# alipay/MMLRec-A-Unified-Multi-Task-and-Multi-Scenario-Learning-Benchmark-for-Recommendation

Measured on AMD Instinct MI355X. Metric: train-step samples/sec, MMoE AliExpress-shape batch, higher is better.
Workload: dtype f32 (GEMMs: fp32-equivalent emulation on the 16-bit MFMA pipe with f32 accumulate -- two scaled fp16 planes per operand where the operand magnitudes travel with the tensors (batches >= 32 768), else three bf16 planes; max-norm error vs float64 3.3e-7 / 4.7e-7, fp32 MFMA 4.3e-7); 1 GPU; mmoe_ae30: 30 sparse fields, 12.49M rows (1e+07-row top table), E=8, mmoe 4 experts, experts [256, 128], gates [64], towers [64], adam lr 0.005; batch_per_gpu=65536, global_batch=65536, index_dist=zipf, table_update=dense_exact, dense_update_schedule=one launch after the scatter, gradients read for marked rows only, hip_graph=True, scatter_mode=deterministic, streams=1, early_fork=0, tables=single GPU

## Files before the change

mmlrec-a-unified-multi-task-and-multi-scenario-learning-benchmark-for-recommendation_amd/csrc/gemm.hip:

```cpp
#include "common.hpp"
#include "gemm_route.hpp"
#include "lds_async.hpp"
#include "reduce.hpp"

#include <stdlib.h>

#include <type_traits>

namespace mml {

using f32x16 = __attribute__((ext_vector_type(16))) float;

constexpr int PITCH_RC = BK + 4;
constexpr int PITCH_NRC = 128 + 4;

struct Source {
  const float* A;
  const float* B;
  int64_t lda, ldb;
  int32_t Kred;
  int32_t vecA, vecB;
  const uint32_t* amaxA;
  const uint32_t* amaxB;
};
// ... 1446 lines not shown
      if (amo) {
        const uint32_t a = lds0 + (uint32_t)(PSTAGES * STG + 256 + tid) * 4u;
        uint32_t v;
        asm volatile("ds_read_b32 %0, %1\n\ts_waitcnt lgkmcnt(0)" : "=v"(v) : "v"(a) : "memory");
        if (v) atomicMax(amo + (blockIdx.x & (MML_AMAX_WORDS - 1)), v);
      }
      uint32_t* const amo2 = K7 ? L.p[tid].amax_out2 : nullptr;
      if (amo2) {
        const uint32_t a = lds0 + (uint32_t)(PSTAGES * STG + 256 + MML_MAX_GROUP + tid) * 4u;
        uint32_t v;
        asm volatile("ds_read_b32 %0, %1\n\ts_waitcnt lgkmcnt(0)" : "=v"(v) : "v"(a) : "memory");
        if (v) atomicMax(amo2 + (blockIdx.x & (MML_AMAX_WORDS - 1)), v);
      }
    }
  }
}

static GemmEnv& gemm_env() {
  static GemmEnv env = [] {
    auto num = [](const char* name, int dflt) {
      const char* e = getenv(name);
      return e ? atoi(e) : dflt;
    };
    auto off = [](const char* name) {
      const char* e = getenv(name);
      return (e && e[0] == '0') ? 0 : 1;
    };
    GemmEnv v = GEMM_ENV_DEFAULT;
    const char* m = getenv("MMLREC_GEMM_MODE");
    v.mode = (m && m[0] >= '0' && m[0] <= '3') ? m[0] - '0' : 4;
    v.panel_on = off("MMLREC_GEMM_PANEL");
    v.ws_on = off("MMLREC_GEMM_WS");
    v.nt_mode = num("MMLREC_GEMM_NT", 1);
    if (v.nt_mode < 0 || v.nt_mode > 3) v.nt_mode = 1;
    v.nt_per_cu = num("MMLREC_NT_PER_CU", 2) == 1 ? 1 : 2;
    v.glds_on = off("MMLREC_GEMM_GLDS");
    v.planes_on = num("MMLREC_GEMM_PLANES", 1);
    v.force_bn = num("MMLREC_GEMM_BN", 0);
    v.wgrad_pad = num("MMLREC_WGRAD_LDS_PAD", 0);
    return v;
  }();
  const char* e = getenv("MMLREC_GEMM_OS");
  env.os_on = (e && e[0] == '0') ? 0 : 1;
  return env;
}

static thread_local char g_last_kernel[96] = "";
static int noted(int rc, const GemmLaunch& g, bool report) {
  if (rc == MML_OK && report) memcpy(g_last_kernel, g.symbol, sizeof(g_last_kernel));
  return rc;
}
static_assert(sizeof(g_last_kernel) == sizeof(GemmLaunch::symbol), "symbol buffers");

template <int EPI, bool A_, bool B_, int N_, bool C_>
static void launch_pipe(const GemmLaunch& G, const Launch& L, hipStream_t st) {
  const dim3 g(G.grid), b(256);
  const size_t dyn = (size_t)G.dyn_lds;
#ifdef MML_LAB
  if (G.bpl) MML_LAUNCH((gemm_pipe_kernel<A_, B_, N_, EPI, MML_LAB_EMU, false, (EPI != EPI_SLAB && MML_LAB_EMU == 2)>), g, b, dyn, st, L);
  else MML_LAUNCH((gemm_pipe_kernel<A_, B_, N_, EPI, MML_LAB_EMU, false>), g, b, dyn, st, L);
#else
  if constexpr (EPI != EPI_SLAB && ((EPI == EPI_FWD) == (B_)) && (EPI == EPI_FWD || N_ == 64)) {
    if (G.k7) {
      if (G.emu == 2 && G.bpl) MML_LAUNCH((gemm_pipe_kernel<A_, B_, N_, EPI, 2, false, true, true>), g, b, dyn, st, L);
      else if (G.emu == 2) MML_LAUNCH((gemm_pipe_kernel<A_, B_, N_, EPI, 2, false, false, true>), g, b, dyn, st, L);
      else MML_LAUNCH((gemm_pipe_kernel<A_, B_, N_, EPI, 3, false, false, true>), g, b, dyn, st, L);
      return;
// ... 45 lines not shown
}

static void put_shape(Problem& P, const TileProb& t) {
  P.M = t.M; P.N = t.N; P.src0 = t.src0; P.nsrc = t.nsrc; P.tiles_n = t.tiles_n; P.tile0 = t.tile0; P.vec_out = t.vec_out;
}
static void put_shape(Source& S, const TileSrc& t) { S.Kred = t.Kred; S.vecA = t.vecA; S.vecB = t.vecB; }

}

using namespace mml;

extern "C" int mml_gemm_set_mode(int32_t mode) {
  MML_REQUIRE(mode == 0 || mode == 1 || mode == 2 || mode == 3 || mode == 4,
              "mml_gemm_set_mode: mode must be 0 (fp32 MFMA), 1 (bf16 operands, reduced precision), 2 / 4 (auto: fp32 "
              "emulated from two scaled fp16 planes where the operand magnitudes are given, else from three bf16 "
              "planes) or 3 (three bf16 planes on every LDS-DMA launch)");
  gemm_env().mode = mode;
  return MML_OK;
}

extern "C" int mml_gemm_get_mode(void) { return gemm_env().mode; }

extern "C" int mml_gemm_set_panel(int32_t on) {
  gemm_env().panel_on = on ? 1 : 0;
  return MML_OK;
}

extern "C" int mml_gemm_set_ws(int32_t on) {
  gemm_env().ws_on = on ? 1 : 0;
  return MML_OK;
}

extern "C" int mml_gemm_set_nt(int32_t on) {
  MML_REQUIRE(on >= 0 && on <= 3, "mml_gemm_set_nt: 0 (off), 1 (every qualifying launch: default), 2 (launches of >= 16 tiles) "
              "or 3 (lab: every qualifying launch on gemm_ntd_kernel)");
  gemm_env().nt_mode = on;
  return MML_OK;
}

extern "C" int mml_gemm_set_wgrad_lds_pad(int32_t bytes) {
  MML_REQUIRE(bytes >= 0 && bytes <= 64 * 1024, "mml_gemm_set_wgrad_lds_pad: bytes outside [0, 65536]");
  gemm_env().wgrad_pad = bytes;
  return MML_OK;
}

extern "C" const char* mml_gemm_last_kernel(void) { return g_last_kernel; }

extern "C" int mml_gemm_nt_serves(const mml_gemm_wgrad_desc* desc) { return (desc && nt_problem_ok(*desc)) ? 1 : 0; }

extern "C" int mml_gemm_os_serves(const mml_gemm_dgrad_desc* d, int32_t n) {
  return (n > 0 && planes_kernels_on(gemm_env()) && os_serves(d, n, gemm_env())) ? 1 : 0;
}

extern "C" int mml_gemm_planes_cut(const mml_planes_desc* d, int32_t n, mml_stream_t stream) {
  MML_REQUIRE(n >= 0 && (n == 0 || d), "mml_gemm_planes_cut: bad descriptor array");
  int i = 0;
  while (i < n) {
    PlanesLaunch L{};
    int64_t items = 0;
    while (i < n && L.n < PLANES_PER_LAUNCH) {
      const mml_planes_desc& q = d[i];
      MML_REQUIRE(q.W && q.planes && q.kexp && q.rows >= 0 && q.cols >= 0 && q.ld >= q.cols,
                  "mml_gemm_planes_cut: matrix %d malformed", i);
      MML_REQUIRE(q.layout == MML_PLANES_ROWS || q.layout == MML_PLANES_COLS, "mml_gemm_planes_cut: layout of matrix %d", i);
      const int64_t ldp = q.ldp ? q.ldp : q.ld;
      MML_REQUIRE(q.layout == MML_PLANES_ROWS ? ldp >= (q.cols + 15) / 16 * 16 : (q.rows % 16 == 0 && ldp >= q.cols),
                  "mml_gemm_planes_cut: matrix %d: the planes pitch cannot hold the reduction extent rounded up to 16 "
                  "(ROWS), or the row count is not a multiple of 16 (COLS)", i);
// ... 227 lines not shown
```

mmlrec-a-unified-multi-task-and-multi-scenario-learning-benchmark-for-recommendation_amd/csrc/gemm_nt.hip:

```cpp
#include "common.hpp"
#include "gemm_route.hpp"
#include "lds_async.hpp"

namespace mml {

typedef float f32x16 __attribute__((ext_vector_type(16)));
typedef short s16x4 __attribute__((ext_vector_type(4)));
typedef short s16x8 __attribute__((ext_vector_type(8)));
typedef __attribute__((address_space(3))) s16x4 lds_s16x4_t;

constexpr int NT_PLANE = NT_STEP * 128;
constexpr int NT_STAGE = 4 * NT_PLANE;

struct NtProblem {
  const float* dC;
  const float* A;
  float* ws;
  float* ws_bias;
  const uint32_t* amax_dc;
  const uint32_t* amax_a;
  int64_t lddc, lda;
  int32_t N, K, ntiles, ktiles;
};
struct NtLaunch {
  NtProblem p[NT_MAX_GROUP];
  int32_t n_prob, steps, slabs, tiles;
};

__device__ __forceinline__ uint32_t nt_amax_load(const uint32_t* p) {
  uint32_t m = 0;
#pragma unroll
  for (int i = 0; i < MML_AMAX_WORDS; ++i) m = p[i] > m ? p[i] : m;
  return m;
}
__device__ __forceinline__ int nt_scale_exp(uint32_t bits) {
  const int e = (int)((bits >> 23) & 0xffu);
  if (e == 255) return 0;
  const int k = 141 - e;
  return k > 110 ? 110 : (k < -110 ? -110 : k);
}
__device__ __forceinline__ float nt_pow2(int k) { return __uint_as_float((uint32_t)(127 + k) << 23); }

__device__ __forceinline__ int nt_swz32(int row) { return ((row & 3) << 2) | ((row >> 2) & 3); }

__device__ __forceinline__ f16x8 nt_frag32(const uint16_t* img, int lo_off, int hi_off) {
  const s16x4 lo = __builtin_amdgcn_ds_read_tr16_b64_v4i16((lds_s16x4_t*)(img + lo_off));
  const s16x4 hi = __builtin_amdgcn_ds_read_tr16_b64_v4i16((lds_s16x4_t*)(img + hi_off));
  const s16x8 v = {lo.x, lo.y, lo.z, lo.w, hi.x, hi.y, hi.z, hi.w};
  return __builtin_bit_cast(f16x8, v);
}
__device__ __forceinline__ int nt_frag_off(int chunk0, int lane, int t) {
  const int g = lane >> 4, hh = g >> 1, q = (lane & 15) >> 2, p = lane & 3;
  const int ch = chunk0 + 2 * (g & 1) + (p >> 1);
  const int row = 8 * hh + 4 * t + q;
  return row * 128 + ((ch ^ nt_swz32(row)) << 3) + 4 * (p & 1);
}

__device__ __forceinline__ void nt_cut4(const float4& x, const float s, uint2& h, uint2& l) {
  typedef float f32x2 __attribute__((ext_vector_type(2)));
  float r0, r1, r2, r3;
  uint32_t h0, h1, l0, l1;
  const f32x2 x01 = {x.x, x.y}, x23 = {x.z, x.w}, ss = {s, s};
  f32x2 y01, y23;
  asm("v_pk_mul_f32 %0, %1, %2" : "=v"(y01) : "v"(x01), "s"(ss));
  asm("v_pk_mul_f32 %0, %1, %2" : "=v"(y23) : "v"(x23), "s"(ss));
  asm("v_cvt_pk_f16_f32 %0, %1, %2" : "=v"(h0) : "v"(y01.x), "v"(y01.y));
  asm("v_cvt_pk_f16_f32 %0, %1, %2" : "=v"(h1) : "v"(y23.x), "v"(y23.y));
  asm("v_fma_mix_f32 %0, %1, %2, -%3 op_sel:[0,0,0] op_sel_hi:[0,0,1]" : "=v"(r0) : "v"(x.x), "s"(s), "v"(h0));
  asm("v_fma_mix_f32 %0, %1, %2, -%3 op_sel:[0,0,1] op_sel_hi:[0,0,1]" : "=v"(r1) : "v"(x.y), "s"(s), "v"(h0));
  asm("v_fma_mix_f32 %0, %1, %2, -%3 op_sel:[0,0,0] op_sel_hi:[0,0,1]" : "=v"(r2) : "v"(x.z), "s"(s), "v"(h1));
  asm("v_fma_mix_f32 %0, %1, %2, -%3 op_sel:[0,0,1] op_sel_hi:[0,0,1]" : "=v"(r3) : "v"(x.w), "s"(s), "v"(h1));
  asm("v_cvt_pk_f16_f32 %0, %1, %2" : "=v"(l0) : "v"(r0), "v"(r1));
  asm("v_cvt_pk_f16_f32 %0, %1, %2" : "=v"(l1) : "v"(r2), "v"(r3));
  h = make_uint2(h0, h1);
  l = make_uint2(l0, l1);
}

__global__ __launch_bounds__(256, 2) void gemm_nt_kernel(const NtLaunch L) {
  __shared__ __attribute__((aligned(16))) uint16_t lds[2 * NT_STAGE];
  const int tid = threadIdx.x, lane = tid & 63, w = __builtin_amdgcn_readfirstlane(tid >> 6);
  const int wn = w >> 1, wk = w & 1;
  const int id = xcd_remap(blockIdx.x, gridDim.x);
  const int slab = id / L.tiles;
  int t = id - slab * L.tiles;
  int pi = 0;
  while (t >= L.p[pi].ntiles * L.p[pi].ktiles) t -= L.p[pi].ntiles * L.p[pi].ktiles, ++pi;
  const NtProblem& P = L.p[pi];
  const int nt = t / P.ktiles, kt = t - nt * P.ktiles;
  const int n0 = nt * 128, k0 = kt * 128;
  const int per = (L.steps + L.slabs - 1) / L.slabs;
  const int s_begin = slab * per, s_end = min(L.steps, s_begin + per);
  const bool want_bias = P.ws_bias != nullptr && kt == 0;

  int kC = nt_scale_exp(nt_amax_load(P.amax_dc)), kA = nt_scale_exp(nt_amax_load(P.amax_a));
  {
    const int over = kC + kA - 126, under = -126 - (kC + kA);
    if (over > 0) { kC -= (over + 1) >> 1; kA -= over >> 1; }
    if (under > 0) { kC += (under + 1) >> 1; kA += under >> 1; }
  }
  kC = __builtin_amdgcn_readfirstlane(kC);
  kA = __builtin_amdgcn_readfirstlane(kA);
  const float sC = nt_pow2(kC), sA = nt_pow2(kA), inv = nt_pow2(-(kC + kA));

  f32x16 acc[2][2];
#pragma unroll
  for (int i = 0; i < 2; ++i)
#pragma unroll
    for (int j = 0; j < 2; ++j)
#pragma unroll
      for (int r = 0; r < 16; ++r) acc[i][j][r] = 0.f;
  float4 bsum = make_float4(0.f, 0.f, 0.f, 0.f);

  const int c4 = tid & 31, r8 = tid >> 5;
  const bool colC = n0 + 4 * c4 < P.N, colA = k0 + 4 * c4 < P.K;
  const uint32_t tC = (uint32_t)(((int64_t)r8 * P.lddc + (colC ? n0 + 4 * c4 : 0)) * 4);
  const uint32_t tA = (uint32_t)(((int64_t)r8 * P.lda + (colA ? k0 + 4 * c4 : 0)) * 4);
  float4 rc0[4], ra0[4], rc1[4], ra1[4];
  const int last = s_end - 1;
  auto load_step = [&](int st, float4 (&rc)[4], float4 (&ra)[4]) __attribute__((always_inline)) {
    st = st > last ? last : st;
    const char* const bC = reinterpret_cast<const char*>(P.dC + (int64_t)st * NT_STEP * P.lddc);
    const char* const bA = reinterpret_cast<const char*>(P.A + (int64_t)st * NT_STEP * P.lda);
#pragma unroll
    for (int p = 0; p < 4; ++p) {
      rc[p] = *reinterpret_cast<const float4*>(bC + (int64_t)(8 * p) * P.lddc * 4 + tC);
      ra[p] = *reinterpret_cast<const float4*>(bA + (int64_t)(8 * p) * P.lda * 4 + tA);
    }
  };
  auto store_step = [&](uint16_t* stage, const float4 (&rc)[4], const float4 (&ra)[4], const float count) __attribute__((always_inline)) {
#pragma unroll
    for (int p = 0; p < 4; ++p) {
      const int row = r8 + 8 * p;
      const int off = row * 128 + (((c4 >> 1) ^ nt_swz32(row)) << 3) + 4 * (c4 & 1);
      uint2 h, l;
      nt_cut4(rc[p], sC, h, l);
      *reinterpret_cast<uint2*>(stage + off) = h;
      *reinterpret_cast<uint2*>(stage + NT_PLANE + off) = l;
      nt_cut4(ra[p], sA, h, l);
      *reinterpret_cast<uint2*>(stage + 2 * NT_PLANE + off) = h;
      *reinterpret_cast<uint2*>(stage + 3 * NT_PLANE + off) = l;
      bsum.x = fmaf(rc[p].x, count, bsum.x); bsum.y = fmaf(rc[p].y, count, bsum.y);
      bsum.z = fmaf(rc[p].z, count, bsum.z); bsum.w = fmaf(rc[p].w, count, bsum.w);
    }
  };
  int offC[2][2], offA[2][2];
#pragma unroll
  for (int i = 0; i < 2; ++i)
#pragma unroll
    for (int t2 = 0; t2 < 2; ++t2) {
      offC[i][t2] = nt_frag_off(wn * 8 + i * 4, lane, t2);
      offA[i][t2] = nt_frag_off(wk * 8 + i * 4, lane, t2);
    }
  auto compute = [&](const uint16_t* cur) __attribute__((always_inline)) {
#pragma unroll
    for (int sub = 0; sub < 2; ++sub) {
      const uint16_t* const b0 = cur + sub * 16 * 128;
      f16x8 ah[2], al[2], bh[2], bl[2];
#pragma unroll
      for (int i = 0; i < 2; ++i) {
        ah[i] = nt_frag32(b0, offC[i][0], offC[i][1]);
        al[i] = nt_frag32(b0 + NT_PLANE, offC[i][0], offC[i][1]);
        bh[i] = nt_frag32(b0 + 2 * NT_PLANE, offA[i][0], offA[i][1]);
        bl[i] = nt_frag32(b0 + 3 * NT_PLANE, offA[i][0], offA[i][1]);
      }
#pragma unroll
      for (int pr = 0; pr < 3; ++pr)
#pragma unroll
        for (int i = 0; i < 2; ++i)
#pragma unroll
          for (int j = 0; j < 2; ++j)
            acc[i][j] = __builtin_amdgcn_mfma_f32_32x32x16_f16(pr == 2 ? al[i] : ah[i], pr == 1 ? bl[j] : bh[j], acc[i][j], 0, 0, 0);
    }
  };

  const int ns = s_end - s_begin;
  if (ns > 0) {
    load_step(s_begin, rc0, ra0);
    load_step(s_begin + 1, rc1, ra1);
    store_step(lds, rc0, ra0, want_bias ? 1.f : 0.f);
  }
  __syncthreads();
#define NT_TRIP(Q, RCL, RAL, RCS, RAS)                                                        \
  {                                                                                           \
    const int q_ = (Q);                                                                       \
    load_step(s_begin + q_ + 2, RCL, RAL);                                                    \
    compute(lds + (q_ & 1) * NT_STAGE);                                                       \
    store_step(lds + ((q_ + 1) & 1) * NT_STAGE, RCS, RAS, (want_bias && q_ + 1 < ns) ? 1.f : 0.f); \
    __syncthreads();                                                                          \
  }
  int q = 0;
  for (; q + 1 < ns; q += 2) {
    NT_TRIP(q, rc0, ra0, rc1, ra1)
    NT_TRIP(q + 1, rc1, ra1, rc0, ra0)
  }
  if (q < ns) NT_TRIP(q, rc0, ra0, rc1, ra1)
#undef NT_TRIP
  bool vi[2], vj[2];
#pragma unroll
  for (int i = 0; i < 2; ++i) {
    vi[i] = n0 + wn * 64 + i * 32 < P.N;
    vj[i] = k0 + wk * 64 + i * 32 < P.K;
  }

  const int h = lane >> 5, c31 = lane & 31;
  float* const ws = P.ws + (int64_t)slab * P.N * P.K;
#pragma unroll
  for (int i = 0; i < 2; ++i)
#pragma unroll
    for (int j = 0; j < 2; ++j) {
      if (!vi[i] || !vj[j]) continue;
      const int k = k0 + wk * 64 + j * 32 + c31;
#pragma unroll
      for (int r = 0; r < 16; ++r) {
        const int n = n0 + wn * 64 + i * 32 + (r & 3) + 8 * (r >> 2) + 4 * h;
        if (k < P.K) ws[(int64_t)n * P.K + k] = acc[i][j][r] * inv;
      }
    }
  if (want_bias) {
    float* const red = reinterpret_cast<float*>(lds);
    *reinterpret_cast<float4*>(red + (r8 * 32 + c4) * 4) = bsum;
    __syncthreads();
    if (tid < 128 && n0 + tid < P.N) {
      float sum = 0.f;
#pragma unroll
      for (int g = 0; g < 8; ++g) sum += red[(g * 32 + (tid >> 2)) * 4 + (tid & 3)];
      P.ws_bias[(int64_t)slab * P.N + n0 + tid] = sum;
    }
  }
}

constexpr int NTD_STAGE = 2 * NT_PLANE;

__global__ __launch_bounds__(256, 2) void gemm_ntd_kernel(const NtLaunch L) {
  __shared__ __attribute__((aligned(16))) uint16_t lds[2 * NTD_STAGE];
  const int tid = threadIdx.x, lane = tid & 63, w = __builtin_amdgcn_readfirstlane(tid >> 6);
  const int wn = w >> 1, wk = w & 1;
  const int id = xcd_remap(blockIdx.x, gridDim.x);
  const int slab = id / L.tiles;
  int t = id - slab * L.tiles;
  int pi = 0;
  while (t >= L.p[pi].ntiles * L.p[pi].ktiles) t -= L.p[pi].ntiles * L.p[pi].ktiles, ++pi;
  const NtProblem& P = L.p[pi];
  const int nt = t / P.ktiles, kt = t - nt * P.ktiles;
  const int n0 = nt * 128, k0 = kt * 128;
  const int per = (L.steps + L.slabs - 1) / L.slabs;
  const int s_begin = slab * per, s_end = min(L.steps, s_begin + per);
  const bool want_bias = P.ws_bias != nullptr && kt == 0;

  int kC = nt_scale_exp(nt_amax_load(P.amax_dc)), kA = nt_scale_exp(nt_amax_load(P.amax_a));
  {
    const int over = kC + kA - 126, under = -126 - (kC + kA);
    if (over > 0) { kC -= (over + 1) >> 1; kA -= over >> 1; }
    if (under > 0) { kC += (under + 1) >> 1; kA += under >> 1; }
  }
  kC = __builtin_amdgcn_readfirstlane(kC);
  kA = __builtin_amdgcn_readfirstlane(kA);
  const float sC = nt_pow2(kC), sA = nt_pow2(kA), inv = nt_pow2(-(kC + kA));

  f32x16 acc[2][2];
#pragma unroll
  for (int i = 0; i < 2; ++i)
#pragma unroll
    for (int j = 0; j < 2; ++j)
#pragma unroll
      for (int r = 0; r < 16; ++r) acc[i][j][r] = 0.f;

  const int c4 = tid & 31, r8 = tid >> 5;
  const bool colA = k0 + 4 * c4 < P.K;
  const uint32_t tA = (uint32_t)(((int64_t)r8 * P.lda + (colA ? k0 + 4 * c4 : 0)) * 4);
  const int hh = lane >> 5, c31 = lane & 31;
  bool vi[2], vj[2];
  uint32_t tD[2];
#pragma unroll
  for (int i = 0; i < 2; ++i) {
    vi[i] = n0 + wn * 64 + i * 32 < P.N;
    vj[i] = k0 + wk * 64 + i * 32 < P.K;
    tD[i] = (uint32_t)(((int64_t)(8 * hh) * P.lddc + (vi[i] ? n0 + wn * 64 + i * 32 : 0) + c31) * 4);
  }
  float bs[2] = {0.f, 0.f};

  float dc0[2][2][8], dc1[2][2][8];
  float4 ra0[4], ra1[4];
  const int last = s_end - 1;
  auto load_step = [&](int st, float (&dc)[2][2][8], float4 (&ra)[4]) __attribute__((always_inline)) {
    st = st > last ? last : st;
    const char* const bC = reinterpret_cast<const char*>(P.dC + (int64_t)st * NT_STEP * P.lddc);
    const char* const bA = reinterpret_cast<const char*>(P.A + (int64_t)st * NT_STEP * P.lda);
#pragma unroll
    for (int sub = 0; sub < 2; ++sub)
#pragma unroll
      for (int e = 0; e < 8; ++e)
#pragma unroll
        for (int i = 0; i < 2; ++i)
          dc[sub][i][e] = *reinterpret_cast<const float*>(bC + (int64_t)(sub * 16 + e) * P.lddc * 4 + tD[i]);
#pragma unroll
    for (int p = 0; p < 4; ++p) ra[p] = *reinterpret_cast<const float4*>(bA + (int64_t)(8 * p) * P.lda * 4 + tA);
  };
  auto store_step = [&](uint16_t* stage, const float4 (&ra)[4]) __attribute__((always_inline)) {
#pragma unroll
    for (int p = 0; p < 4; ++p) {
      const int row = r8 + 8 * p;
      const int off = row * 128 + (((c4 >> 1) ^ nt_swz32(row)) << 3) + 4 * (c4 & 1);
      uint2 h, l;
      nt_cut4(ra[p], sA, h, l);
      *reinterpret_cast<uint2*>(stage + off) = h;
      *reinterpret_cast<uint2*>(stage + NT_PLANE + off) = l;
    }
  };
  int offA[2][2];
#pragma unroll
  for (int i = 0; i < 2; ++i)
#pragma unroll
    for (int t2 = 0; t2 < 2; ++t2) offA[i][t2] = nt_frag_off(wk * 8 + i * 4, lane, t2);
  auto compute = [&](const uint16_t* cur, const float (&dc)[2][2][8]) __attribute__((always_inline)) {
#pragma unroll
    for (int sub = 0; sub < 2; ++sub) {
      const uint16_t* const b0 = cur + sub * 16 * 128;
      f16x8 ah[2], al[2], bh[2], bl[2];
#pragma unroll
      for (int i = 0; i < 2; ++i) {
        bh[i] = nt_frag32(b0, offA[i][0], offA[i][1]);
        bl[i] = nt_frag32(b0 + NT_PLANE, offA[i][0], offA[i][1]);
      }
#pragma unroll
      for (int i = 0; i < 2; ++i) {
        const float4 x0 = make_float4(dc[sub][i][0], dc[sub][i][1], dc[sub][i][2], dc[sub][i][3]);
        const float4 x1 = make_float4(dc[sub][i][4], dc[sub][i][5], dc[sub][i][6], dc[sub][i][7]);
// ... 8 lines not shown
#pragma unroll
      for (int pr = 0; pr < 3; ++pr)
#pragma unroll
        for (int i = 0; i < 2; ++i)
#pragma unroll
          for (int j = 0; j < 2; ++j)
            acc[i][j] = __builtin_amdgcn_mfma_f32_32x32x16_f16(pr == 2 ? al[i] : ah[i], pr == 1 ? bl[j] : bh[j], acc[i][j], 0, 0, 0);
    }
  };

  const int ns = s_end - s_begin;
  if (ns > 0) {
    load_step(s_begin, dc0, ra0);
    load_step(s_begin + 1, dc1, ra1);
    store_step(lds, ra0);
  }
  __syncthreads();
#define NTD_TRIP(Q, DCQ, RAQ, RAS)                                                            \
  {                                                                                           \
    const int q_ = (Q);                                                                       \
    compute(lds + (q_ & 1) * NTD_STAGE, DCQ);                                                 \
    store_step(lds + ((q_ + 1) & 1) * NTD_STAGE, RAS);                                        \
    load_step(s_begin + q_ + 2, DCQ, RAQ);                                                    \
    __syncthreads();                                                                          \
  }
  int q = 0;
  for (; q + 1 < ns; q += 2) {
    NTD_TRIP(q, dc0, ra0, ra1)
    NTD_TRIP(q + 1, dc1, ra1, ra0)
  }
  if (q < ns) NTD_TRIP(q, dc0, ra0, ra1)
#undef NTD_TRIP

  float* const ws = P.ws + (int64_t)slab * P.N * P.K;
#pragma unroll
  for (int i = 0; i < 2; ++i)
#pragma unroll
    for (int j = 0; j < 2; ++j) {
      if (!vi[i] || !vj[j]) continue;
      const int k = k0 + wk * 64 + j * 32 + c31;
#pragma unroll
      for (int r = 0; r < 16; ++r) {
        const int n = n0 + wn * 64 + i * 32 + (r & 3) + 8 * (r >> 2) + 4 * hh;
        if (k < P.K) ws[(int64_t)n * P.K + k] = acc[i][j][r] * inv;
      }
    }
  if (want_bias) {
#pragma unroll
    for (int i = 0; i < 2; ++i) {
      const float sum = bs[i] + __shfl_xor(bs[i], 32, 64);
      if (wk == 0 && hh == 0 && vi[i]) P.ws_bias[(int64_t)slab * P.N + n0 + wn * 64 + i * 32 + c31] = sum;
    }
  }
}

struct NtRedProblem {
  const float* ws;
  const float* ws_bias;
  float* dW;
  float* dbias;
  int64_t lddw;
  int32_t N, K, accumulate;
};
struct NtRedLaunch {
  NtRedProblem p[NT_MAX_GROUP];
  int32_t n_prob, slabs;
};
__global__ __launch_bounds__(256) void nt_reduce_kernel(const NtRedLaunch L) {
  __shared__ float4 part[4][64];
  const NtRedProblem& P = L.p[blockIdx.y];
  const int k4 = P.K >> 2;
  const int64_t total = (int64_t)P.N * k4;
  const int64_t plane = (int64_t)P.N * P.K;
  const int e = threadIdx.x & 63, g = threadIdx.x >> 6;
  const int per = (L.slabs + 3) >> 2;
  const int s0 = g * per, s1 = min(L.slabs, s0 + per);
  for (int64_t base = (int64_t)blockIdx.x * 64; base < total; base += (int64_t)gridDim.x * 64) {
    const int64_t it = base + e;
    float4 s = make_float4(0.f, 0.f, 0.f, 0.f);
    int64_t n = 0;
    int k = 0;
    if (it < total) {
      n = it / k4;
      k = (int)(it - n * k4) * 4;
      const float* const src = P.ws + n * P.K + k;
// ... 25 lines not shown
    __syncthreads();
  }
  if (P.dbias && blockIdx.x == 0) {
    for (int n = threadIdx.x; n < P.N; n += blockDim.x) {
      float s = P.ws_bias[n];
      int sl = 1;
      for (; sl + 8 <= L.slabs; sl += 8) {
        float v[8];
#pragma unroll
        for (int u = 0; u < 8; ++u) v[u] = P.ws_bias[(int64_t)(sl + u) * P.N + n];
#pragma unroll
        for (int u = 0; u < 8; ++u) s += v[u];
      }
      for (; sl < L.slabs; ++sl) s += P.ws_bias[(int64_t)sl * P.N + n];
      P.dbias[n] = P.accumulate ? P.dbias[n] + s : s;
    }
  }
}

}

using namespace mml;

int mml_gemm_nt_launch(const mml_gemm_wgrad_desc* d, const GemmLaunch& g, void* workspace, hipStream_t st) {
  NtLaunch L{};
  NtRedLaunch R{};
  const int n = g.count;
  const int64_t slabs = g.slabs;
  L.n_prob = R.n_prob = n;
  L.steps = d[0].M / NT_STEP;
  L.slabs = R.slabs = g.slabs;
  float* ws = reinterpret_cast<float*>(workspace);
  int maxred = 1;
  for (int i = 0; i < n; ++i) {
    const mml_gemm_wgrad_desc& q = d[i];
    NtProblem& P = L.p[i];
    P.dC = q.dC; P.A = q.A; P.lddc = q.lddc; P.lda = q.lda; P.N = q.N; P.K = q.K;
    P.amax_dc = q.amax_dc; P.amax_a = q.amax_a;
    P.ntiles = (int)cdiv(q.N, 128); P.ktiles = (int)cdiv(q.K, 128);
    P.ws = ws;
    ws += slabs * q.N * q.K;
    P.ws_bias = q.dbias ? ws : nullptr;
    ws += slabs * q.N;
    L.tiles += P.ntiles * P.ktiles;
    NtRedProblem& Q = R.p[i];
    Q.ws = P.ws; Q.ws_bias = P.ws_bias; Q.dW = q.dW; Q.dbias = q.dbias; Q.lddw = q.lddw; Q.N = q.N; Q.K = q.K;
    Q.accumulate = q.accumulate;
    const int blocks = (int)cdiv((int64_t)q.N * q.K / 4, 64);
    maxred = blocks > maxred ? blocks : maxred;
  }
  if (g.partials) {
    if (g.ntd) MML_LAUNCH(gemm_ntd_kernel, dim3(g.grid), dim3(256), (size_t)g.dyn_lds, st, L);
    else MML_LAUNCH(gemm_nt_kernel, dim3(g.grid), dim3(256), (size_t)g.dyn_lds, st, L);
    const int rc = check_launch("mml_gemm_grouped_wgrad(nt)");
    if (rc != MML_OK) return rc;
  }
  if (g.reduce) {
    if (maxred > 2048) maxred = 2048;
    MML_LAUNCH(nt_reduce_kernel, dim3((unsigned)maxred, (unsigned)n), dim3(256), 0, st, R);
    return check_launch("mml_gemm_grouped_wgrad(nt reduce)");
  }
  return MML_OK;
}
```

mmlrec-a-unified-multi-task-and-multi-scenario-learning-benchmark-for-recommendation_amd/csrc/gemm_route.hpp:

```cpp
#pragma once
#include <stdint.h>

#include "../../include/mmlrec.h"

namespace mml {

struct GemmEnv {
  int mode;
  int panel_on;
  int ws_on;
  int os_on;
  int nt_mode;
  int nt_per_cu;
  int glds_on;
  int planes_on;
  int force_bn;
  int wgrad_pad;
};
constexpr GemmEnv GEMM_ENV_DEFAULT = {4, 1, 1, 1, 1, 2, 1, 1, 0, 0};

constexpr int BM = 128;
constexpr int BK = 32;
constexpr int GK = 16;
constexpr int MAX_SOURCES = 24;
// ... 4 lines not shown
constexpr int WS_W_BYTES = 128 * 1024;
constexpr int WS_MIN_ROWS = 8192;
constexpr int ws_dgroup(const int kred) { return kred <= 0 ? 0 : (kred % 64 == 0 ? 4 : (kred % 80 == 0 ? 5 : 0)); }
constexpr int OS_BM = 256;
constexpr int OS_NC = 256;
constexpr int NT_MAX_GROUP = 48;
constexpr int NT_STEP = 32;
constexpr int NT_MIN_TILES = 16;

enum GemmFamily { GEMM_PANEL, GEMM_WS, GEMM_OS, GEMM_NT, GEMM_PIPE, GEMM_REG };

struct TileSrc {
  int32_t Kred, vecA, vecB;
};
struct TileProb {
  int32_t M, N, src0, nsrc;
  int32_t tiles_m, tiles_n, tile0, vec_out;
};

struct GemmLaunch {
  int family;
  int first, count;
  uint32_t grid;
  int32_t dyn_lds;
  char symbol[96];
  bool arc, brc, bcols, bpl, k7, masks;
  int bn, epi, emu;
  int32_t rows, row0;
  int nout, dgroup, n_prob, wg_per_prob;
  uint8_t member[MML_MAX_GROUP];
  int slabs;
  int64_t tiles;
  bool ntd;
  TileSrc s[MAX_SOURCES];
  TileProb p[MML_MAX_GROUP];
  int32_t total_ntiles, tiles_m;
  bool partials, reduce;
  int32_t S, chunk;
  int64_t slab_floats, ws_off;
};

struct GemmRefusal {
  int code;
  char msg[256];
};

struct RouteText {
  char* s;
  int cap, n;
  RouteText(char* buf, int c) : s(buf), cap(c), n(0) { s[0] = 0; }
  RouteText& operator<<(const char* t) {
    while (*t && n + 1 < cap) s[n++] = *t++;
    s[n] = 0;
    return *this;
  }
  RouteText& operator<<(long long v) {
    char dg[24];
    int k = 0;
    unsigned long long u = v < 0 ? 0ull - (unsigned long long)v : (unsigned long long)v;
    do dg[k++] = (char)('0' + u % 10); while (u /= 10);
    if (v < 0) dg[k++] = '-';
    while (k && n + 1 < cap) s[n++] = dg[--k];
    s[n] = 0;
    return *this;
  }
  RouteText& operator<<(int v) { return *this << (long long)v; }
// ... 149 lines not shown
  }
  return MML_OK;
}

inline bool os_serves(const mml_gemm_dgrad_desc* d, int n, const GemmEnv& env) {
  if (!env.os_on || !d || n != 1) return false;
  const mml_gemm_dgrad_desc& q = d[0];
  if (q.gate_h || q.Y || q.relu_mask || q.act != MML_ACT_NONE || !q.dA) return false;
  if (q.n_src < 2 || q.n_src > MML_MAX_SRC) return false;
  if (q.M < 16384 || q.K < 192 || q.K > OS_NC || q.K % 4 != 0) return false;
  if (!route_al16(q.dA) || q.ldda % 4 != 0 || q.ldda < q.K) return false;
  if ((int64_t)q.M * q.ldda >= (1ll << 40)) return false;
  int64_t ntot = 0;
  for (int s = 0; s < q.n_src; ++s) {
    if (q.w_kn[s] != 0 || !q.dC[s] || !q.w_planes[s] || !q.w_kexp[s] || !q.amax_dc[s]) return false;
    if (q.w_kexp[s] != q.w_kexp[0]) return false;
    if (q.N[s] <= 0 || q.N[s] % 16 != 0) return false;
    if (!route_al16(q.dC[s]) || q.lddc[s] % 4 != 0 || q.lddc[s] < q.N[s]) return false;
    if (!route_al16(q.w_planes[s]) || q.ldw[s] % 4 != 0 || q.ldw[s] < q.K) return false;
    ntot += q.N[s];
  }
  return ntot >= 256;
}

inline bool nt_problem_ok(const mml_gemm_wgrad_desc& q) {
  if (q.M < 16384 || q.M % NT_STEP != 0) return false;
  if (q.w_kn || !q.dC || !q.A || !q.dW || !q.amax_dc || !q.amax_a) return false;
  if (q.N <= 0 || q.N % 32 != 0 || q.K <= 0 || q.K % 4 != 0) return false;
  if (!route_al16(q.dC) || !route_al16(q.A) || q.lddc % 4 != 0 || q.lda % 4 != 0 || q.lddc < q.N || q.lda < q.K ||
      q.lddw < q.K)
    return false;
  return true;
}
inline bool nt_serves(const mml_gemm_wgrad_desc* d, int n, int64_t workspace_bytes, const GemmEnv& env, int cus,
                      GemmLaunch& g) {
  if (env.nt_mode == 0 || n < 1 || n > NT_MAX_GROUP) return false;
  const int32_t M = d[0].M;
  if (M < 16384 || M % NT_STEP != 0) return false;
  int64_t tiles = 0, elems = 0;
  for (int i = 0; i < n; ++i) {
    const mml_gemm_wgrad_desc& q = d[i];
    if (q.M != M || !nt_problem_ok(q)) return false;
    tiles += route_cdiv(q.N, 128) * route_cdiv(q.K, 128);
    elems += (int64_t)q.N * q.K + q.N;
  }
  if (env.nt_mode == 2 && tiles < NT_MIN_TILES) return false;
  const int steps = M / NT_STEP;
  int64_t slabs = (env.nt_per_cu * (int64_t)cus) / tiles;
  if (slabs > steps / 8) slabs = steps / 8;
  if (slabs > 64) slabs = 64;
  const int64_t fit = workspace_bytes / (elems * 4);
  if (slabs > fit) slabs = fit;
  if (slabs < 1) return false;
  g.family = GEMM_NT;
  g.first = 0;
  g.count = n;
  g.slabs = (int)slabs;
  g.tiles = tiles;
  g.grid = (uint32_t)(tiles * slabs);
  g.ntd = env.nt_mode == 3;
  g.dyn_lds = (env.nt_per_cu == 1 && !g.ntd) ? 20480 : 0;
  return true;
}

inline void pick_tiles(const int32_t* Ns, int n, int64_t row_tiles, const GemmEnv& env, int& bn, int& emu) {
#ifdef MML_LAB
  bn = MML_LAB_BN;
  emu = MML_LAB_EMU;
  return;
#endif
  int64_t pad64 = 0, pad128 = 0;
  for (int i = 0; i < n; ++i) {
    pad64 += route_cdiv(Ns[i], 64) * 64;
    pad128 += route_cdiv(Ns[i], 128) * 128;
  }
  bn = (pad128 * 100 <= pad64 * 150) ? 128 : 64;
  if (row_tiles * (pad128 / 128) < 1024) bn = 64;
  if (env.force_bn == 64 || env.force_bn == 128) bn = env.force_bn;
  emu = (env.mode == 0) ? 0 : (env.mode == 1 ? 1 : 3);
}

inline bool pipe_ok(const GemmLaunch& g, const GemmEnv& env) {
  if (!env.glds_on) return false;
  for (int i = 0; i < g.count; ++i) {
    const TileProb& P = g.p[i];
    if (!g.arc && (P.M % 4 != 0 || P.M < 4)) return false;
    if (!g.brc && (P.N % 4 != 0 || P.N < 4)) return false;
    if (P.M < 1 || P.N < 1) return false;
    for (int s = 0; s < P.nsrc; ++s) {
      const TileSrc& S = g.s[P.src0 + s];
      if (S.Kred % GK != 0 || S.Kred < GK || !S.vecA || !S.vecB) return false;
    }
  }
// ... 391 lines not shown
```

Before: 61.89 million samples/s.

## Pair half-filled NT wgrad tiles from problems sharing the same A operand

The weight-gradient NT kernel now pairs problems whose last N tile is at most half full and that share the same A input. Each warp half stages and computes its own problem's dC slice against the shared A tile. This is meant to cut wasted MFMA work and redundant A loads on half-empty 128-wide tiles, and the smaller tile count can also raise the slab count. When the two problems need different A scales, the kernel runs two passes, which adds extra loads, syncs and more complex control flow. Mode 4 turns pairing off for A/B comparison.

```diff
diff --git a/mmlrec-a-unified-multi-task-and-multi-scenario-learning-benchmark-for-recommendation_amd/csrc/gemm.hip b/mmlrec-a-unified-multi-task-and-multi-scenario-learning-benchmark-for-recommendation_amd/csrc/gemm.hip
--- a/mmlrec-a-unified-multi-task-and-multi-scenario-learning-benchmark-for-recommendation_amd/csrc/gemm.hip
+++ b/mmlrec-a-unified-multi-task-and-multi-scenario-learning-benchmark-for-recommendation_amd/csrc/gemm.hip
@@ -1502,7 +1502,7 @@
     v.panel_on = off("MMLREC_GEMM_PANEL");
     v.ws_on = off("MMLREC_GEMM_WS");
     v.nt_mode = num("MMLREC_GEMM_NT", 1);
-    if (v.nt_mode < 0 || v.nt_mode > 3) v.nt_mode = 1;
+    if (v.nt_mode < 0 || v.nt_mode > 4) v.nt_mode = 1;
     v.nt_per_cu = num("MMLREC_NT_PER_CU", 2) == 1 ? 1 : 2;
     v.glds_on = off("MMLREC_GEMM_GLDS");
     v.planes_on = num("MMLREC_GEMM_PLANES", 1);
@@ -1614,8 +1614,8 @@
 }
 
 extern "C" int mml_gemm_set_nt(int32_t on) {
-  MML_REQUIRE(on >= 0 && on <= 3, "mml_gemm_set_nt: 0 (off), 1 (every qualifying launch: default), 2 (launches of >= 16 tiles) "
-              "or 3 (lab: every qualifying launch on gemm_ntd_kernel)");
+  MML_REQUIRE(on >= 0 && on <= 4, "mml_gemm_set_nt: 0 (off), 1 (every qualifying launch: default), 2 (launches of >= 16 tiles), "
+              "3 (lab: every qualifying launch on gemm_ntd_kernel) or 4 (A/B: as 1, half tiles unpaired)");
   gemm_env().nt_mode = on;
   return MML_OK;
 }
diff --git a/mmlrec-a-unified-multi-task-and-multi-scenario-learning-benchmark-for-recommendation_amd/csrc/gemm_nt.hip b/mmlrec-a-unified-multi-task-and-multi-scenario-learning-benchmark-for-recommendation_amd/csrc/gemm_nt.hip
--- a/mmlrec-a-unified-multi-task-and-multi-scenario-learning-benchmark-for-recommendation_amd/csrc/gemm_nt.hip
+++ b/mmlrec-a-unified-multi-task-and-multi-scenario-learning-benchmark-for-recommendation_amd/csrc/gemm_nt.hip
@@ -12,19 +12,9 @@
 constexpr int NT_PLANE = NT_STEP * 128;
 constexpr int NT_STAGE = 4 * NT_PLANE;
 
-struct NtProblem {
-  const float* dC;
-  const float* A;
-  float* ws;
-  float* ws_bias;
-  const uint32_t* amax_dc;
-  const uint32_t* amax_a;
-  int64_t lddc, lda;
-  int32_t N, K, ntiles, ktiles;
-};
-struct NtLaunch {
-  NtProblem p[NT_MAX_GROUP];
-  int32_t n_prob, steps, slabs, tiles;
+template <bool B>
+struct NtFlag {
+  static constexpr bool value = B;
 };
 
 __device__ __forceinline__ uint32_t nt_amax_load(const uint32_t* p) {
@@ -87,62 +77,33 @@
   while (t >= L.p[pi].ntiles * L.p[pi].ktiles) t -= L.p[pi].ntiles * L.p[pi].ktiles, ++pi;
   const NtProblem& P = L.p[pi];
   const int nt = t / P.ktiles, kt = t - nt * P.ktiles;
-  const int n0 = nt * 128, k0 = kt * 128;
+  const int k0 = kt * 128;
   const int per = (L.steps + L.slabs - 1) / L.slabs;
   const int s_begin = slab * per, s_end = min(L.steps, s_begin + per);
-  const bool want_bias = P.ws_bias != nullptr && kt == 0;
-
-  int kC = nt_scale_exp(nt_amax_load(P.amax_dc)), kA = nt_scale_exp(nt_amax_load(P.amax_a));
-  {
+  const bool paired = P.partner >= 0 && nt == ((P.N - 1) >> 7);
+  const NtProblem& Q = L.p[paired ? P.partner : pi];
+  const NtProblem& X = wn ? Q : P;
+  const int nb = paired ? (wn ? ((Q.N - 1) >> 7) * 128 : nt * 128) : nt * 128 + wn * 64;
+
+  const int kA0 = nt_scale_exp(nt_amax_load(P.amax_a));
+  int kCs[2], kAs[2];
+#pragma unroll
+  for (int hf = 0; hf < 2; ++hf) {
+    int kC = nt_scale_exp(nt_amax_load(hf ? Q.amax_dc : P.amax_dc)), kA = kA0;
     const int over = kC + kA - 126, under = -126 - (kC + kA);
     if (over > 0) { kC -= (over + 1) >> 1; kA -= over >> 1; }
     if (under > 0) { kC += (under + 1) >> 1; kA += under >> 1; }
-  }
-  kC = __builtin_amdgcn_readfirstlane(kC);
-  kA = __builtin_amdgcn_readfirstlane(kA);
-  const float sC = nt_pow2(kC), sA = nt_pow2(kA), inv = nt_pow2(-(kC + kA));
-
-  f32x16 acc[2][2];
-#pragma unroll
-  for (int i = 0; i < 2; ++i)
-#pragma unroll
-    for (int j = 0; j < 2; ++j)
-#pragma unroll
-      for (int r = 0; r < 16; ++r) acc[i][j][r] = 0.f;
-  float4 bsum = make_float4(0.f, 0.f, 0.f, 0.f);
-
-  const int c4 = tid & 31, r8 = tid >> 5;
-  const bool colC = n0 + 4 * c4 < P.N, colA = k0 + 4 * c4 < P.K;
-  const uint32_t tC = (uint32_t)(((int64_t)r8 * P.lddc + (colC ? n0 + 4 * c4 : 0)) * 4);
-  const uint32_t tA = (uint32_t)(((int64_t)r8 * P.lda + (colA ? k0 + 4 * c4 : 0)) * 4);
-  float4 rc0[4], ra0[4], rc1[4], ra1[4];
-  const int last = s_end - 1;
-  auto load_step = [&](int st, float4 (&rc)[4], float4 (&ra)[4]) __attribute__((always_inline)) {
-    st = st > last ? last : st;
-    const char* const bC = reinterpret_cast<const char*>(P.dC + (int64_t)st * NT_STEP * P.lddc);
-    const char* const bA = reinterpret_cast<const char*>(P.A + (int64_t)st * NT_STEP * P.lda);
-#pragma unroll
-    for (int p = 0; p < 4; ++p) {
-      rc[p] = *reinterpret_cast<const float4*>(bC + (int64_t)(8 * p) * P.lddc * 4 + tC);
-      ra[p] = *reinterpret_cast<const float4*>(bA + (int64_t)(8 * p) * P.lda * 4 + tA);
-    }
-  };
-  auto store_step = [&](uint16_t* stage, const float4 (&rc)[4], const float4 (&ra)[4], const float count) __attribute__((always_inline)) {
-#pragma unroll
-    for (int p = 0; p < 4; ++p) {
-      const int row = r8 + 8 * p;
-      const int off = row * 128 + (((c4 >> 1) ^ nt_swz32(row)) << 3) + 4 * (c4 & 1);
-      uint2 h, l;
-      nt_cut4(rc[p], sC, h, l);
-      *reinterpret_cast<uint2*>(stage + off) = h;
-      *reinterpret_cast<uint2*>(stage + NT_PLANE + off) = l;
-      nt_cut4(ra[p], sA, h, l);
-      *reinterpret_cast<uint2*>(stage + 2 * NT_PLANE + off) = h;
-      *reinterpret_cast<uint2*>(stage + 3 * NT_PLANE + off) = l;
-      bsum.x = fmaf(rc[p].x, count, bsum.x); bsum.y = fmaf(rc[p].y, count, bsum.y);
-      bsum.z = fmaf(rc[p].z, count, bsum.z); bsum.w = fmaf(rc[p].w, count, bsum.w);
-    }
-  };
+    kCs[hf] = __builtin_amdgcn_readfirstlane(kC);
+    kAs[hf] = __builtin_amdgcn_readfirstlane(kA);
+  }
+  const bool split = kAs[0] != kAs[1];
+  const int kC = wn ? kCs[1] : kCs[0], kAx = wn ? kAs[1] : kAs[0];
+  const float sC = nt_pow2(kC), inv = nt_pow2(-(kC + kAx));
+
+  const int c16 = lane & 15, r8 = wk * 4 + (lane >> 4);
+  const bool colC = nb + 4 * c16 < X.N, colA = k0 + wn * 64 + 4 * c16 < P.K;
+  const uint32_t tC = (uint32_t)(((int64_t)r8 * X.lddc + (colC ? nb + 4 * c16 : 0)) * 4);
+  const uint32_t tA = (uint32_t)(((int64_t)r8 * P.lda + (colA ? k0 + wn * 64 + 4 * c16 : 0)) * 4);
   int offC[2][2], offA[2][2];
 #pragma unroll
   for (int i = 0; i < 2; ++i)
@@ -151,6 +112,52 @@
       offC[i][t2] = nt_frag_off(wn * 8 + i * 4, lane, t2);
       offA[i][t2] = nt_frag_off(wk * 8 + i * 4, lane, t2);
     }
+  const int ns = s_end - s_begin, last = s_end - 1;
+  const int h = lane >> 5, c31 = lane & 31;
+
+  auto run_pass = [&](const int pass) __attribute__((always_inline)) {
+  const bool stage = nb < X.N && (!split || wn == pass);
+  const bool active = stage && k0 + wk * 64 < P.K;
+  const bool want_bias = stage && X.ws_bias != nullptr && kt == 0;
+  const float sA = nt_pow2(pass ? kAs[1] : kAs[0]);
+
+  f32x16 acc[2][2];
+#pragma unroll
+  for (int i = 0; i < 2; ++i)
+#pragma unroll
+    for (int j = 0; j < 2; ++j)
+#pragma unroll
+      for (int r = 0; r < 16; ++r) acc[i][j][r] = 0.f;
+  float4 bsum = make_float4(0.f, 0.f, 0.f, 0.f);
+  float4 rc0[4], ra0[4], rc1[4], ra1[4];
+  auto load_step = [&](auto sc, int st, float4 (&rc)[4], float4 (&ra)[4]) __attribute__((always_inline)) {
+    st = st > last ? last : st;
+    const char* const bC = reinterpret_cast<const char*>(X.dC + (int64_t)st * NT_STEP * X.lddc);
+    const char* const bA = reinterpret_cast<const char*>(P.A + (int64_t)st * NT_STEP * P.lda);
+#pragma unroll
+    for (int p = 0; p < 4; ++p) {
+      if constexpr (decltype(sc)::value) rc[p] = *reinterpret_cast<const float4*>(bC + (int64_t)(8 * p) * X.lddc * 4 + tC);
+      ra[p] = *reinterpret_cast<const float4*>(bA + (int64_t)(8 * p) * P.lda * 4 + tA);
+    }
+  };
+  auto store_step = [&](auto sc, uint16_t* stg, const float4 (&rc)[4], const float4 (&ra)[4], const float count) __attribute__((always_inline)) {
+#pragma unroll
+    for (int p = 0; p < 4; ++p) {
+      const int row = r8 + 8 * p;
+      const int off = row * 128 + (((wn * 8 + (c16 >> 1)) ^ nt_swz32(row)) << 3) + 4 * (c16 & 1);
+      uint2 hp, lp;
+      if constexpr (decltype(sc)::value) {
+        nt_cut4(rc[p], sC, hp, lp);
+        *reinterpret_cast<uint2*>(stg + off) = hp;
+        *reinterpret_cast<uint2*>(stg + NT_PLANE + off) = lp;
+        bsum.x = fmaf(rc[p].x, count, bsum.x); bsum.y = fmaf(rc[p].y, count, bsum.y);
+        bsum.z = fmaf(rc[p].z, count, bsum.z); bsum.w = fmaf(rc[p].w, count, bsum.w);
+      }
+      nt_cut4(ra[p], sA, hp, lp);
+      *reinterpret_cast<uint2*>(stg + 2 * NT_PLANE + off) = hp;
+      *reinterpret_cast<uint2*>(stg + 3 * NT_PLANE + off) = lp;
+    }
+  };
   auto compute = [&](const uint16_t* cur) __attribute__((always_inline)) {
 #pragma unroll
     for (int sub = 0; sub < 2; ++sub) {
@@ -173,59 +180,64 @@
     }
   };
 
-  const int ns = s_end - s_begin;
-  if (ns > 0) {
-    load_step(s_begin, rc0, ra0);
-    load_step(s_begin + 1, rc1, ra1);
-    store_step(lds, rc0, ra0, want_bias ? 1.f : 0.f);
-  }
-  __syncthreads();
-#define NT_TRIP(Q, RCL, RAL, RCS, RAS)                                                        \
-  {                                                                                           \
-    const int q_ = (Q);                                                                       \
-    load_step(s_begin + q_ + 2, RCL, RAL);                                                    \
-    compute(lds + (q_ & 1) * NT_STAGE);                                                       \
-    store_step(lds + ((q_ + 1) & 1) * NT_STAGE, RCS, RAS, (want_bias && q_ + 1 < ns) ? 1.f : 0.f); \
-    __syncthreads();                                                                          \
-  }
-  int q = 0;
-  for (; q + 1 < ns; q += 2) {
-    NT_TRIP(q, rc0, ra0, rc1, ra1)
-    NT_TRIP(q + 1, rc1, ra1, rc0, ra0)
-  }
-  if (q < ns) NT_TRIP(q, rc0, ra0, rc1, ra1)
+#define NT_TRIP(SC, ACT, Q, RCL, RAL, RCS, RAS)                                                        \
+  {                                                                                                    \
+    const int q_ = (Q);                                                                                \
+    load_step(SC, s_begin + q_ + 2, RCL, RAL);                                                         \
+    if constexpr (decltype(ACT)::value) compute(lds + (q_ & 1) * NT_STAGE);                            \
+    store_step(SC, lds + ((q_ + 1) & 1) * NT_STAGE, RCS, RAS, (want_bias && q_ + 1 < ns) ? 1.f : 0.f); \
+    __syncthreads();                                                                                   \
+  }
+  auto walk = [&](auto sc, auto act) __attribute__((always_inline)) {
+    if (ns > 0) {
+      load_step(sc, s_begin, rc0, ra0);
+      load_step(sc, s_begin + 1, rc1, ra1);
+      store_step(sc, lds, rc0, ra0, want_bias ? 1.f : 0.f);
+    }
+    __syncthreads();
+    int q = 0;
+    for (; q + 1 < ns; q += 2) {
+      NT_TRIP(sc, act, q, rc0, ra0, rc1, ra1)
+      NT_TRIP(sc, act, q + 1, rc1, ra1, rc0, ra0)
+    }
+    if (q < ns) NT_TRIP(sc, act, q, rc0, ra0, rc1, ra1)
+  };
+  if (active) walk(NtFlag<true>{}, NtFlag<true>{});
+  else if (stage) walk(NtFlag<true>{}, NtFlag<false>{});
+  else walk(NtFlag<false>{}, NtFlag<false>{});
 #undef NT_TRIP
-  bool vi[2], vj[2];
-#pragma unroll
-  for (int i = 0; i < 2; ++i) {
-    vi[i] = n0 + wn * 64 + i * 32 < P.N;
-    vj[i] = k0 + wk * 64 + i * 32 < P.K;
-  }
-
-  const int h = lane >> 5, c31 = lane & 31;
-  float* const ws = P.ws + (int64_t)slab * P.N * P.K;
-#pragma unroll
-  for (int i = 0; i < 2; ++i)
-#pragma unroll
-    for (int j = 0; j < 2; ++j) {
-      if (!vi[i] || !vj[j]) continue;
-      const int k = k0 + wk * 64 + j * 32 + c31;
-#pragma unroll
-      for (int r = 0; r < 16; ++r) {
-        const int n = n0 + wn * 64 + i * 32 + (r & 3) + 8 * (r >> 2) + 4 * h;
-        if (k < P.K) ws[(int64_t)n * P.K + k] = acc[i][j][r] * inv;
-      }
-    }
-  if (want_bias) {
+
+  if (active) {
+    float* const ws = X.ws + (int64_t)slab * X.N * X.K;
+#pragma unroll
+    for (int i = 0; i < 2; ++i)
+#pragma unroll
+      for (int j = 0; j < 2; ++j) {
+        if (nb + i * 32 >= X.N || k0 + wk * 64 + j * 32 >= X.K) continue;
+        const int k = k0 + wk * 64 + j * 32 + c31;
+#pragma unroll
+        for (int r = 0; r < 16; ++r) {
+          const int n = nb + i * 32 + (r & 3) + 8 * (r >> 2) + 4 * h;
+          if (k < X.K) ws[(int64_t)n * X.K + k] = acc[i][j][r] * inv;
+        }
+      }
+  }
+  if (kt == 0 && (P.ws_bias != nullptr || Q.ws_bias != nullptr)) {
     float* const red = reinterpret_cast<float*>(lds);
-    *reinterpret_cast<float4*>(red + (r8 * 32 + c4) * 4) = bsum;
+    *reinterpret_cast<float4*>(red + (r8 * 32 + wn * 16 + c16) * 4) = bsum;
     __syncthreads();
-    if (tid < 128 && n0 + tid < P.N) {
+    if (want_bias && wk == 0 && nb + lane < X.N) {
       float sum = 0.f;
 #pragma unroll
-      for (int g = 0; g < 8; ++g) sum += red[(g * 32 + (tid >> 2)) * 4 + (tid & 3)];
-      P.ws_bias[(int64_t)slab * P.N + n0 + tid] = sum;
-    }
+      for (int g = 0; g < 8; ++g) sum += red[(g * 32 + wn * 16 + (lane >> 2)) * 4 + (lane & 3)];
+      X.ws_bias[(int64_t)slab * X.N + nb + lane] = sum;
+    }
+  }
+  };
+  run_pass(0);
+  if (split) {
+    __syncthreads();
+    run_pass(1);
   }
 }
 
@@ -242,20 +254,32 @@
   while (t >= L.p[pi].ntiles * L.p[pi].ktiles) t -= L.p[pi].ntiles * L.p[pi].ktiles, ++pi;
   const NtProblem& P = L.p[pi];
   const int nt = t / P.ktiles, kt = t - nt * P.ktiles;
-  const int n0 = nt * 128, k0 = kt * 128;
+  const int k0 = kt * 128;
   const int per = (L.steps + L.slabs - 1) / L.slabs;
   const int s_begin = slab * per, s_end = min(L.steps, s_begin + per);
-  const bool want_bias = P.ws_bias != nullptr && kt == 0;
-
-  int kC = nt_scale_exp(nt_amax_load(P.amax_dc)), kA = nt_scale_exp(nt_amax_load(P.amax_a));
-  {
+  const bool paired = P.partner >= 0 && nt == ((P.N - 1) >> 7);
+  const NtProblem& Q = L.p[paired ? P.partner : pi];
+  const NtProblem& X = wn ? Q : P;
+  const int nb = paired ? (wn ? ((Q.N - 1) >> 7) * 128 : nt * 128) : nt * 128 + wn * 64;
+  const int kA0 = nt_scale_exp(nt_amax_load(P.amax_a));
+  int kCs[2], kAs[2];
+#pragma unroll
+  for (int hf = 0; hf < 2; ++hf) {
+    int kC = nt_scale_exp(nt_amax_load(hf ? Q.amax_dc : P.amax_dc)), kA = kA0;
     const int over = kC + kA - 126, under = -126 - (kC + kA);
     if (over > 0) { kC -= (over + 1) >> 1; kA -= over >> 1; }
     if (under > 0) { kC += (under + 1) >> 1; kA += under >> 1; }
-  }
-  kC = __builtin_amdgcn_readfirstlane(kC);
-  kA = __builtin_amdgcn_readfirstlane(kA);
-  const float sC = nt_pow2(kC), sA = nt_pow2(kA), inv = nt_pow2(-(kC + kA));
+    kCs[hf] = __builtin_amdgcn_readfirstlane(kC);
+    kAs[hf] = __builtin_amdgcn_readfirstlane(kA);
+  }
+  const bool split = kAs[0] != kAs[1];
+  const int kCx = wn ? kCs[1] : kCs[0], kAx = wn ? kAs[1] : kAs[0];
+  const float sC = nt_pow2(kCx), inv = nt_pow2(-(kCx + kAx));
+
+  auto run_pass = [&](const int pass) __attribute__((always_inline)) {
+  const bool mine = !split || wn == pass;
+  const bool want_bias = mine && X.ws_bias != nullptr && kt == 0;
+  const float sA = nt_pow2(pass ? kAs[1] : kAs[0]);
 
   f32x16 acc[2][2];
 #pragma unroll
@@ -273,9 +297,9 @@
   uint32_t tD[2];
 #pragma unroll
   for (int i = 0; i < 2; ++i) {
-    vi[i] = n0 + wn * 64 + i * 32 < P.N;
+    vi[i] = nb + i * 32 < X.N;
     vj[i] = k0 + wk * 64 + i * 32 < P.K;
-    tD[i] = (uint32_t)(((int64_t)(8 * hh) * P.lddc + (vi[i] ? n0 + wn * 64 + i * 32 : 0) + c31) * 4);
+    tD[i] = (uint32_t)(((int64_t)(8 * hh) * X.lddc + (vi[i] ? nb + i * 32 : 0) + c31) * 4);
   }
   float bs[2] = {0.f, 0.f};
 
@@ -284,7 +308,7 @@
   const int last = s_end - 1;
   auto load_step = [&](int st, float (&dc)[2][2][8], float4 (&ra)[4]) __attribute__((always_inline)) {
     st = st > last ? last : st;
-    const char* const bC = reinterpret_cast<const char*>(P.dC + (int64_t)st * NT_STEP * P.lddc);
+    const char* const bC = reinterpret_cast<const char*>(X.dC + (int64_t)st * NT_STEP * X.lddc);
     const char* const bA = reinterpret_cast<const char*>(P.A + (int64_t)st * NT_STEP * P.lda);
 #pragma unroll
     for (int sub = 0; sub < 2; ++sub)
@@ -292,7 +316,7 @@
       for (int e = 0; e < 8; ++e)
 #pragma unroll
         for (int i = 0; i < 2; ++i)
-          dc[sub][i][e] = *reinterpret_cast<const float*>(bC + (int64_t)(sub * 16 + e) * P.lddc * 4 + tD[i]);
+          dc[sub][i][e] = *reinterpret_cast<const float*>(bC + (int64_t)(sub * 16 + e) * X.lddc * 4 + tD[i]);
 #pragma unroll
     for (int p = 0; p < 4; ++p) ra[p] = *reinterpret_cast<const float4*>(bA + (int64_t)(8 * p) * P.lda * 4 + tA);
   };
@@ -367,25 +391,31 @@
   if (q < ns) NTD_TRIP(q, dc0, ra0, ra1)
 #undef NTD_TRIP
 
-  float* const ws = P.ws + (int64_t)slab * P.N * P.K;
+  float* const ws = X.ws + (int64_t)slab * X.N * X.K;
 #pragma unroll
   for (int i = 0; i < 2; ++i)
 #pragma unroll
     for (int j = 0; j < 2; ++j) {
-      if (!vi[i] || !vj[j]) continue;
+      if (!mine || !vi[i] || !vj[j]) continue;
       const int k = k0 + wk * 64 + j * 32 + c31;
 #pragma unroll
       for (int r = 0; r < 16; ++r) {
-        const int n = n0 + wn * 64 + i * 32 + (r & 3) + 8 * (r >> 2) + 4 * hh;
-        if (k < P.K) ws[(int64_t)n * P.K + k] = acc[i][j][r] * inv;
+        const int n = nb + i * 32 + (r & 3) + 8 * (r >> 2) + 4 * hh;
+        if (k < X.K) ws[(int64_t)n * X.K + k] = acc[i][j][r] * inv;
       }
     }
   if (want_bias) {
 #pragma unroll
     for (int i = 0; i < 2; ++i) {
       const float sum = bs[i] + __shfl_xor(bs[i], 32, 64);
-      if (wk == 0 && hh == 0 && vi[i]) P.ws_bias[(int64_t)slab * P.N + n0 + wn * 64 + i * 32 + c31] = sum;
-    }
+      if (wk == 0 && hh == 0 && vi[i]) X.ws_bias[(int64_t)slab * X.N + nb + i * 32 + c31] = sum;
+    }
+  }
+  };
+  run_pass(0);
+  if (split) {
+    __syncthreads();
+    run_pass(1);
   }
 }
 
@@ -477,17 +507,19 @@
   L.slabs = R.slabs = g.slabs;
   float* ws = reinterpret_cast<float*>(workspace);
   int maxred = 1;
+  NtPlan plan;
+  nt_plan(d, n, g.pairing, plan);
+  L.tiles = (int32_t)plan.tiles;
   for (int i = 0; i < n; ++i) {
     const mml_gemm_wgrad_desc& q = d[i];
     NtProblem& P = L.p[i];
     P.dC = q.dC; P.A = q.A; P.lddc = q.lddc; P.lda = q.lda; P.N = q.N; P.K = q.K;
     P.amax_dc = q.amax_dc; P.amax_a = q.amax_a;
-    P.ntiles = (int)cdiv(q.N, 128); P.ktiles = (int)cdiv(q.K, 128);
+    P.ntiles = plan.ntiles[i]; P.ktiles = plan.ktiles[i]; P.partner = plan.partner[i];
     P.ws = ws;
     ws += slabs * q.N * q.K;
     P.ws_bias = q.dbias ? ws : nullptr;
     ws += slabs * q.N;
-    L.tiles += P.ntiles * P.ktiles;
     NtRedProblem& Q = R.p[i];
     Q.ws = P.ws; Q.ws_bias = P.ws_bias; Q.dW = q.dW; Q.dbias = q.dbias; Q.lddw = q.lddw; Q.N = q.N; Q.K = q.K;
     Q.accumulate = q.accumulate;
diff --git a/mmlrec-a-unified-multi-task-and-multi-scenario-learning-benchmark-for-recommendation_amd/csrc/gemm_route.hpp b/mmlrec-a-unified-multi-task-and-multi-scenario-learning-benchmark-for-recommendation_amd/csrc/gemm_route.hpp
--- a/mmlrec-a-unified-multi-task-and-multi-scenario-learning-benchmark-for-recommendation_amd/csrc/gemm_route.hpp
+++ b/mmlrec-a-unified-multi-task-and-multi-scenario-learning-benchmark-for-recommendation_amd/csrc/gemm_route.hpp
@@ -60,6 +60,8 @@
   int slabs;
   int64_t tiles;
   bool ntd;
+  bool pairing;
+  int pairs;
   TileSrc s[MAX_SOURCES];
   TileProb p[MML_MAX_GROUP];
   int32_t total_ntiles, tiles_m;
@@ -275,18 +277,69 @@
     return false;
   return true;
 }
+struct NtPlan {
+  int16_t partner[NT_MAX_GROUP];
+  uint16_t ntiles[NT_MAX_GROUP];
+  uint16_t ktiles[NT_MAX_GROUP];
+  int64_t tiles;
+  int32_t pairs;
+};
+inline bool nt_half_tile(const mml_gemm_wgrad_desc& q) { return (q.N - 1) % 128 < 64; }
+inline bool nt_pairable(const mml_gemm_wgrad_desc& a, const mml_gemm_wgrad_desc& b) {
+  return nt_half_tile(a) && nt_half_tile(b) && a.A == b.A && a.lda == b.lda && a.K == b.K && a.amax_a == b.amax_a &&
+         a.M == b.M;
+}
+inline void nt_plan(const mml_gemm_wgrad_desc* d, int n, bool pairing, NtPlan& p) {
+  bool second[NT_MAX_GROUP] = {};
+  p.tiles = 0;
+  p.pairs = 0;
+  for (int i = 0; i < n; ++i) p.partner[i] = -1;
+  for (int i = 0; i < n; ++i) {
+    for (int j = i + 1; pairing && !second[i] && p.partner[i] < 0 && j < n; ++j)
+      if (!second[j] && p.partner[j] < 0 && nt_pairable(d[i], d[j])) {
+        p.partner[i] = (int16_t)j;
+        second[j] = true;
+        ++p.pairs;
+      }
+    p.ntiles[i] = (uint16_t)(route_cdiv(d[i].N, 128) - (second[i] ? 1 : 0));
+    p.ktiles[i] = (uint16_t)route_cdiv(d[i].K, 128);
+    p.tiles += (int64_t)p.ntiles[i] * p.ktiles[i];
+  }
+}
+struct NtProblem {
+  const float* dC;
+  const float* A;
+  float* ws;
+  float* ws_bias;
+  const uint32_t* amax_dc;
+  const uint32_t* amax_a;
+  int64_t lddc, lda;
+  int32_t N, K;
+  uint16_t ntiles, ktiles;
+  int16_t partner, pad;
+};
+struct NtLaunch {
+  NtProblem p[NT_MAX_GROUP];
+  int32_t n_prob, steps, slabs, tiles;
+};
+static_assert(sizeof(NtLaunch) <= 4096, "gemm_nt_kernel's descriptor must fit the 4 KiB kernel-argument block");
+inline bool nt_pairing(const GemmEnv& env) { return env.nt_mode != 4; }
+
 inline bool nt_serves(const mml_gemm_wgrad_desc* d, int n, int64_t workspace_bytes, const GemmEnv& env, int cus,
                       GemmLaunch& g) {
   if (env.nt_mode == 0 || n < 1 || n > NT_MAX_GROUP) return false;
   const int32_t M = d[0].M;
   if (M < 16384 || M % NT_STEP != 0) return false;
-  int64_t tiles = 0, elems = 0;
+  int64_t elems = 0;
   for (int i = 0; i < n; ++i) {
     const mml_gemm_wgrad_desc& q = d[i];
     if (q.M != M || !nt_problem_ok(q)) return false;
-    tiles += route_cdiv(q.N, 128) * route_cdiv(q.K, 128);
+    if (q.N > 128 * 65535 || q.K > 128 * 65535) return false;
     elems += (int64_t)q.N * q.K + q.N;
   }
+  NtPlan plan;
+  nt_plan(d, n, nt_pairing(env), plan);
+  const int64_t tiles = plan.tiles;
   if (env.nt_mode == 2 && tiles < NT_MIN_TILES) return false;
   const int steps = M / NT_STEP;
   int64_t slabs = (env.nt_per_cu * (int64_t)cus) / tiles;
@@ -302,6 +355,8 @@
   g.tiles = tiles;
   g.grid = (uint32_t)(tiles * slabs);
   g.ntd = env.nt_mode == 3;
+  g.pairing = nt_pairing(env);
+  g.pairs = plan.pairs;
   g.dyn_lds = (env.nt_per_cu == 1 && !g.ntd) ? 20480 : 0;
   return true;
 }
```

New measurement: 61.73 million samples/s. Within noise of the previous version (-0.3%).
